# domkirke/acids_transforms

Hardware: AMD Instinct MI355X
Metric: spectrogram frames/sec (fwd+invert), n_fft=1024 hop=256 (higher is better)
Workload: dtype f32; 1 GPU; configs[1]: batch=1024 clips/GPU x 4 s mono 44.1 kHz, STFT fwd + Magnitude(mel=128, log1p, unipolar) [one fused kernel] + ISTFT invert, fp32; n_fft=1024, hop=256, frames_per_clip=690, clips_per_gpu=1024

## Files before the change

acids_transforms_amd/csrc/capi.hip:

```cpp
#include <hip/hip_runtime.h>
#include <math.h>
#include <stdint.h>
#include <vector>

#include "../../include/acids_hip.h"
#include "autograd.h"
#include "band_bank.h"
#include "fft512.h"
#include "stft_launch.h"

#include <atomic>
#include "variants.h"
namespace at_hip {
constexpr int kMaxDevices = 16;
static float2* g_twiddles[kMaxDevices] = {nullptr};
static float2* g_side[kMaxDevices] = {nullptr};

static bool device_tables(const float2*& tw, const float2*& side) {
  int dev = 0;
  if (hipGetDevice(&dev) != hipSuccess || dev < 0 || dev >= kMaxDevices || !g_twiddles[dev]) return false;
  tw = g_twiddles[dev];
  side = g_side[dev];
  return true;
}

static bool is_pow2(int n) { return n > 0 && (n & (n - 1)) == 0; }
static bool fft_size_ok(int n) { return n >= 2 && n <= 16384 && (!(n & 1) || n < 8192); }
static bool fft_mixed(int n) { return !is_pow2(n) || n < 8; }

__global__ void envelope_table_kernel(const float* w, int n_fft, int hop, int R, float* env) {
  int i = blockIdx.x * blockDim.x + threadIdx.x;
  if (i >= (1 << R) * hop) return;
  int mask = i / hop, r = i - mask * hop;
  float s = 0.f;
  for (int q = 0; q < R; ++q)
    if (mask & (1 << q)) {
      int o = hop * (R - 1 - q) + r;
      if (o < n_fft) s += w[o] * w[o];
    }
  env[i] = s;
}
static std::atomic<int> g_variants[kVarCount];
int variant(int which) { return g_variants[which].load(std::memory_order_relaxed); }
}

using namespace at_hip;

extern "C" {

int at_abi_version(void) { return 4; }

int at_set_variant(int which, int value) {
  if (which < 0 || which >= kVarCount || value < 0 || value > (which >= kVarFirstPlan ? 65535 : 4)) return AT_EINVAL;
  g_variants[which].store(value, std::memory_order_relaxed);
  return AT_OK;
}

int at_get_variant(int which) {
  if (which < 0 || which >= kVarCount) return AT_EINVAL;
  return g_variants[which].load(std::memory_order_relaxed);
}

const char* at_error_string(int code) {
  switch (code) {
    case AT_OK: return "ok";
    case AT_EINVAL: return "invalid argument";
    case AT_EUNSUPPORTED: return "unsupported configuration";
    case AT_ENOTINIT: return "at_init() not called for this device";
    case AT_EWORKSPACE: return "workspace too small";
    case AT_ELAUNCH: return "HIP launch/runtime error";
    default: return "unknown error";
  }
}

int at_init(int device) {
  if (device < 0 || device >= kMaxDevices) return AT_EINVAL;
  if (g_twiddles[device]) return AT_OK;
  int prev = 0;
  if (hipGetDevice(&prev) != hipSuccess) return AT_ELAUNCH;
  if (hipSetDevice(device) != hipSuccess) return AT_ELAUNCH;
  std::vector<float2> tab(kTwiddleCount);
  const double two_pi = 6.283185307179586476925286766559;
  for (int k = 1; k < 8; ++k)
    for (int l = 0; l < 64; ++l) {
      double a1 = -two_pi * (double)(l * k) / 512.0;
      tab[(k - 1) * 64 + l] = make_float2((float)cos(a1), (float)sin(a1));
      double a2 = -two_pi * (double)((l & 7) * k) / 64.0;
      tab[(7 + k - 1) * 64 + l] = make_float2((float)cos(a2), (float)sin(a2));
    }
  for (int m = 0; m < 8; ++m)
    for (int l = 0; l < 64; ++l) {
      double a = -two_pi * (double)(l + 64 * m) / 1024.0;
      tab[(14 + m) * 64 + l] = make_float2((float)cos(a), (float)sin(a));
    }
  float2* d = nullptr;
  int rc = AT_OK;
  if (hipMalloc((void**)&d, sizeof(float2) * (kTwiddleCount + kTileCtrSlots)) != hipSuccess) rc = AT_ELAUNCH;
  if (rc == AT_OK && hipMemcpy(d, tab.data(), sizeof(float2) * kTwiddleCount, hipMemcpyHostToDevice) != hipSuccess)
    rc = AT_ELAUNCH;
  if (rc == AT_OK && hipMemset(d + kTwiddleCount, 0, sizeof(float2) * kTileCtrSlots) != hipSuccess) rc = AT_ELAUNCH;
  float2* d2 = nullptr;
  if (rc == AT_OK) {
    std::vector<float2> t2(kSideTableCount);
    auto fill = [&](int at, int count, int r, double n) {
      for (int k = 0; k < count; ++k) {
        const double a = -two_pi * (double)(r * k) / n;
        t2[at + k] = make_float2((float)cos(a), (float)sin(a));
      }
    };
    fill(kSideW2048, 1024, 1, 2048.0);
    fill(kSideW512, 256, 1, 512.0);
    for (int r = 1; r < 4; ++r) fill(kSide256 + (r - 1) * 128, 128, r, 512.0);
    for (int r = 1; r < 8; ++r) fill(kSide128 + (r - 1) * 64, 64, r, 512.0);
    fill(kSide4096, 2048, 1, 4096.0);
    for (int r = 1; r < 4; ++r) fill(kSide4096Radix + (r - 1) * 512, 512, r, 2048.0);
    if (hipMalloc((void**)&d2, sizeof(float2) * t2.size()) != hipSuccess) rc = AT_ELAUNCH;
    if (rc == AT_OK && hipMemcpy(d2, t2.data(), sizeof(float2) * t2.size(), hipMemcpyHostToDevice) != hipSuccess)
      rc = AT_ELAUNCH;
  }
  if (rc == AT_OK) {
    g_side[device] = d2;
    g_twiddles[device] = d;
  }
  (void)hipSetDevice(prev);
  return rc;
}

int at_stft_forward(const float* x, int64_t B, int64_t L, int64_t clip_stride, int64_t T, int n_fft, int hop,
                    int center, const float* window, float* out_complex, float* phase, void* stream) {
  if (B < 0 || T < 0 || L < 0 || hop <= 0 || n_fft <= 0) return AT_EINVAL;
  if (B * T == 0) return AT_OK;
  if (!x || !window || !out_complex) return AT_EINVAL;
  if (!fft_size_ok(n_fft)) return AT_EUNSUPPORTED;
  if (center && L <= n_fft / 2) return AT_EINVAL;
  hipStream_t s = (hipStream_t)stream;
  const uintptr_t walign = (uintptr_t)window;
  const float2 *tw = nullptr, *side = nullptr;
  if (n_fft == 1024 && (walign & 7) == 0) {
    if (!device_tables(tw, side)) return AT_ENOTINIT;
    if ((hop == 256 || hop == 128 || hop == 512) && center && (clip_stride & 1) == 0)
      return launch_stft1024_h256_fwd(x, B, L, clip_stride, T, window, tw, (float2*)out_complex, phase, nullptr,
                                      nullptr, nullptr, nullptr, 0.f, 0, 0, 0, s, nullptr, hop);
    return launch_stft1024_fwd(x, B, L, clip_stride, T, hop, center, window, tw, (float2*)out_complex, phase, s);
  }
  if (n_fft == 2048 && (walign & 15) == 0) {
    if (!device_tables(tw, side)) return AT_ENOTINIT;
    return launch_stft2048_fwd(x, B, L, clip_stride, T, hop, center, window, tw, side + kSideW2048, (float2*)out_complex,
                               phase, s);
  }
  if (n_fft == 4096 && (walign & 15) == 0) {
    if (!device_tables(tw, side)) return AT_ENOTINIT;
    return launch_stft4096_fwd(x, B, L, clip_stride, T, hop, center, window, tw, side + kSide4096, (float2*)out_complex,
                               phase, s);
  }
  if ((n_fft == 256 || n_fft == 128) && (walign & 7) == 0) {
    if (!device_tables(tw, side)) return AT_ENOTINIT;
    return launch_stft_small_fwd(n_fft, x, B, L, clip_stride, T, hop, center, window, tw,
                                 side + (n_fft == 256 ? kSide256 : kSide128), (float2*)out_complex, phase, s);
  }
  if (n_fft == 512 && (walign & 7) == 0) {
    if (!device_tables(tw, side)) return AT_ENOTINIT;
    return launch_stft512_fwd(x, B, L, clip_stride, T, hop, center, window, tw, side + kSideW512, (float2*)out_complex,
                              phase, s);
  }
  if (fft_mixed(n_fft))
    return launch_rfft_mixed(x, B, L, clip_stride, T, n_fft, hop, center, window, (float2*)out_complex, phase, s);
  return launch_rfft_generic(x, B, L, clip_stride, T, n_fft, hop, center, window, (float2*)out_complex, phase, s);
}

int at_stft_mel_forward(const float* x, int64_t B, int64_t L, int64_t clip_stride, int64_t T, int n_fft, int hop,
                        const float* window, const int32_t* lane_filter, const int32_t* lane_start,
                        const float* band_weights, int n_filters, int n_passes, const int32_t* pass_len_host,
                        int contrast, int power2, const float* offset, const float* scale, float eps,
                        float* out_complex_or_null, float* phase_or_null, float* feat, int feat_channel_major,
                        void* stream) {
  if (B < 0 || T < 0 || L < 0) return AT_EINVAL;
// ... 403 lines not shown
```

acids_transforms_amd/csrc/fft512.h:

```cpp
#pragma once
#include <hip/hip_runtime.h>
#include <stdint.h>

#include "fastmath.h"

namespace at_hip {

#ifndef AT_WAVE_PRIORITY
#define AT_WAVE_PRIORITY 1
#endif
template <int LEVEL>
__device__ __forceinline__ void wave_priority() {
#if AT_WAVE_PRIORITY
  __builtin_amdgcn_s_setprio(LEVEL);
#endif
}

constexpr int kFftLdsFloat2PerWave = 568;

constexpr int kTwiddleCount = 22 * 64;
constexpr int kTileCtrSlots = 4096;

__device__ __forceinline__ float2 cadd(float2 a, float2 b) { return make_float2(a.x + b.x, a.y + b.y); }

typedef float v2f __attribute__((ext_vector_type(2)));

__device__ __forceinline__ v2f to_v(float2 a) { return (v2f){a.x, a.y}; }
__device__ __forceinline__ float2 to_f2(v2f a) { return make_float2(a.x, a.y); }

__device__ __forceinline__ v2f add_mi(v2f a, v2f b) {
  v2f r;
  asm("v_pk_add_f32 %0, %1, %2 op_sel:[0,1] op_sel_hi:[1,0] neg_hi:[0,1]" : "=v"(r) : "v"(a), "v"(b));
  return r;
}
__device__ __forceinline__ v2f add_pi(v2f a, v2f b) {
  v2f r;
  asm("v_pk_add_f32 %0, %1, %2 op_sel:[0,1] op_sel_hi:[1,0] neg_lo:[0,1]" : "=v"(r) : "v"(a), "v"(b));
  return r;
}
__device__ __forceinline__ v2f fma_mi(v2f a, v2f b, v2f rr) {
  v2f r;
  asm("v_pk_fma_f32 %0, %1, %2, %3 op_sel:[1,0,0] op_sel_hi:[0,1,1] neg_hi:[1,0,0]" : "=v"(r) : "v"(b), "s"(rr), "v"(a));
  return r;
}
__device__ __forceinline__ v2f fma_pi(v2f a, v2f b, v2f rr) {
  v2f r;
  asm("v_pk_fma_f32 %0, %1, %2, %3 op_sel:[1,0,0] op_sel_hi:[0,1,1] neg_lo:[1,0,0]" : "=v"(r) : "v"(b), "s"(rr), "v"(a));
  return r;
}
template <bool INV> __device__ __forceinline__ v2f rot_add(v2f a, v2f b) { return INV ? add_pi(a, b) : add_mi(a, b); }
template <bool INV> __device__ __forceinline__ v2f rot_sub(v2f a, v2f b) { return INV ? add_mi(a, b) : add_pi(a, b); }
template <bool INV> __device__ __forceinline__ v2f rot_fma(v2f a, v2f b, v2f rr) { return INV ? fma_pi(a, b, rr) : fma_mi(a, b, rr); }
template <bool INV> __device__ __forceinline__ v2f rot_fms(v2f a, v2f b, v2f rr) { return INV ? fma_mi(a, b, rr) : fma_pi(a, b, rr); }

__device__ __forceinline__ v2f cmul_v(v2f a, v2f w) {
  const v2f t = a.yy * w.yx;
  v2f r;
  asm("v_pk_fma_f32 %0, %1, %2, %3 op_sel_hi:[0,1,1] neg_lo:[0,0,1]" : "=v"(r) : "v"(a), "v"(w), "v"(t));
  return r;
}
__device__ __forceinline__ v2f cmul_conj_v(v2f a, v2f w) {
  const v2f t = a.yy * w.yx;
  v2f r;
  asm("v_pk_fma_f32 %0, %1, %2, %3 op_sel_hi:[0,1,1] neg_hi:[0,1,0]" : "=v"(r) : "v"(a), "v"(w), "v"(t));
  return r;
}
template <bool INV> __device__ __forceinline__ v2f twiddle(v2f a, v2f w) { return INV ? cmul_conj_v(a, w) : cmul_v(a, w); }
__device__ __forceinline__ v2f add_conj(v2f a, v2f b) {
  v2f r;
  asm("v_pk_add_f32 %0, %1, %2 neg_hi:[0,1]" : "=v"(r) : "v"(a), "v"(b));
  return r;
}
__device__ __forceinline__ v2f sub_conj(v2f a, v2f b) {
  v2f r;
  asm("v_pk_add_f32 %0, %1, %2 neg_lo:[0,1]" : "=v"(r) : "v"(a), "v"(b));
  return r;
}
__device__ __forceinline__ v2f scale_add_mi(v2f a, v2f hh, v2f b) {
  v2f r;
  asm("v_pk_fma_f32 %0, %1, %2, %3 op_sel:[0,0,1] op_sel_hi:[1,1,0] neg_hi:[0,0,1]" : "=v"(r) : "v"(a), "s"(hh), "v"(b));
  return r;
}

template <bool INV>
__device__ __forceinline__ void radix8(v2f (&v)[8]) {
  const v2f rr = {0.70710678118654752440f, 0.70710678118654752440f};
  const v2f a0 = v[0] + v[4], a4 = v[0] - v[4];
  const v2f a1 = v[1] + v[5], d1 = v[1] - v[5];
  const v2f a2 = v[2] + v[6], d2 = v[2] - v[6];
  const v2f a3 = v[3] + v[7], d3 = v[3] - v[7];
  const v2f s5 = rot_add<INV>(d1, d1);
  const v2f s7 = rot_sub<INV>(d3, d3);
  const v2f b0 = a0 + a2, b2 = a0 - a2;
  const v2f b1 = a1 + a3, d13 = a1 - a3;
  const v2f b4 = rot_add<INV>(a4, d2), b6 = rot_sub<INV>(a4, d2);
  const v2f u5 = s5 - s7, u7 = s5 + s7;
  v[0] = b0 + b1;
  v[4] = b0 - b1;
  v[2] = rot_add<INV>(b2, d13);
  v[6] = rot_sub<INV>(b2, d13);
  v[1] = __builtin_elementwise_fma(u5, rr, b4);
  v[5] = __builtin_elementwise_fma(-u5, rr, b4);
  v[3] = rot_fma<INV>(b6, u7, rr);
  v[7] = rot_fms<INV>(b6, u7, rr);
}

#ifndef AT_LDS_NOMERGE
#define AT_LDS_NOMERGE 1
#endif
template <typename T>
__device__ __forceinline__ T lds_read_single(const T* p) {
#if AT_LDS_NOMERGE
  typedef const volatile __attribute__((address_space(3))) T* lds_ptr;
  return *(lds_ptr)(p);
#else
  return *p;
#endif
}

__device__ __forceinline__ void wave_lds_sync() {
  __builtin_amdgcn_fence(__ATOMIC_RELEASE, "wavefront");
  __builtin_amdgcn_wave_barrier();
  __builtin_amdgcn_fence(__ATOMIC_ACQUIRE, "wavefront");
}

struct Twiddles {
  v2f t1[7];
  v2f t2[7];
  v2f tr[8];
  __device__ __forceinline__ v2f get1(int k) const { return t1[k]; }
  __device__ __forceinline__ v2f get2(int k) const { return t2[k]; }
  __device__ __forceinline__ v2f getr(int m) const { return tr[m]; }
};

template <bool INV>
struct LdsTwiddles {
  const float2* tab;
  int lane;
  __device__ __forceinline__ v2f get1(int k) const { return lds_read_single(reinterpret_cast<const v2f*>(tab) + k * 64 + lane); }
  __device__ __forceinline__ v2f get2(int k) const { return lds_read_single(reinterpret_cast<const v2f*>(tab) + (7 + k) * 64 + lane); }
  __device__ __forceinline__ v2f getr(int m) const { return lds_read_single(reinterpret_cast<const v2f*>(tab) + (14 + m) * 64 + lane); }
};
struct HybridTwiddles {
  v2f t1[7];
  v2f t2[7];
  const float2* tab;
  int col;
  __device__ __forceinline__ v2f get1(int k) const { return t1[k]; }
  __device__ __forceinline__ v2f get2(int k) const { return t2[k]; }
  __device__ __forceinline__ v2f getr(int m) const { return lds_read_single(reinterpret_cast<const v2f*>(tab) + (14 + m) * 64 + col); }
};

template <bool INV>
__device__ __forceinline__ float2 twiddle_for_lds(const float2* __restrict__ tab, int i) {
  const float2 a = tab[i];
  return (!INV && i >= 14 * 64) ? make_float2(0.5f * a.x, 0.5f * a.y) : a;
}

template <bool INV>
__device__ __forceinline__ void load_twiddles(Twiddles& tw, const float2* __restrict__ tab, int lane) {
#pragma unroll
  for (int k = 0; k < 7; ++k) {
    tw.t1[k] = to_v(tab[k * 64 + lane]);
    tw.t2[k] = to_v(tab[(7 + k) * 64 + lane]);
  }
#pragma unroll
  for (int m = 0; m < 8; ++m) tw.tr[m] = to_v(twiddle_for_lds<INV>(tab, (14 + m) * 64 + lane));
}

#ifndef AT_XCHG1_SWAP
#define AT_XCHG1_SWAP 1
#endif
__device__ __forceinline__ void xchg1_registers(v2f (&v)[8]) {
#pragma unroll
  for (int k = 0; k < 4; ++k)
#pragma unroll
    for (int c = 0; c < 2; ++c) {
      const auto sw = __builtin_amdgcn_permlane32_swap(__float_as_uint(v[k][c]), __float_as_uint(v[k + 4][c]), false, false);
      v[k][c] = __uint_as_float(sw[0]);
      v[k + 4][c] = __uint_as_float(sw[1]);
    }
#pragma unroll
  for (int g = 0; g < 8; g += 4)
#pragma unroll
    for (int k = g; k < g + 2; ++k)
#pragma unroll
      for (int c = 0; c < 2; ++c) {
        const auto sw = __builtin_amdgcn_permlane16_swap(__float_as_uint(v[k][c]), __float_as_uint(v[k + 2][c]), false, false);
        v[k][c] = __uint_as_float(sw[0]);
        v[k + 2][c] = __uint_as_float(sw[1]);
      }
#pragma unroll
  for (int k = 0; k < 8; k += 2)
#pragma unroll
    for (int c = 0; c < 2; ++c) {
      const int a = __float_as_int(v[k][c]), b = __float_as_int(v[k + 1][c]);
      const int a2 = __builtin_amdgcn_update_dpp(a, b, 0x128, 0xf, 0xc, false);
      const int b2 = __builtin_amdgcn_update_dpp(b, a, 0x128, 0xf, 0x3, false);
      v[k][c] = __int_as_float(a2);
      v[k + 1][c] = __int_as_float(b2);
    }
}

template <bool INV, typename TW>
__device__ __forceinline__ void fft512(v2f (&v)[8], const TW& tw, float2* lds_f2, int lane, int out_lane = -1) {
  if (out_lane < 0) out_lane = lane;
  v2f* lds = reinterpret_cast<v2f*>(lds_f2);
  const int lo = lane & 7, hi = lane >> 3;
  radix8<INV>(v);
#pragma unroll
  for (int k = 1; k < 8; ++k) v[k] = twiddle<INV>(v[k], tw.get1(k - 1));
  if constexpr (AT_XCHG1_SWAP == 2 || (AT_XCHG1_SWAP == 1 && !INV)) {
    xchg1_registers(v);
  } else {
#pragma unroll
    for (int k = 0; k < 8; ++k) lds[hi * 72 + lo + 8 * k] = v[k];
    wave_lds_sync();
#pragma unroll
    for (int k = 0; k < 8; ++k) v[k] = lds_read_single(lds + k * 72 + lane);
    wave_lds_sync();
  }
  radix8<INV>(v);
#pragma unroll
  for (int k = 1; k < 8; ++k) v[k] = twiddle<INV>(v[k], tw.get2(k - 1));
#pragma unroll
  for (int k = 0; k < 8; ++k) lds[lo * 66 + hi + 8 * k] = v[k];
  wave_lds_sync();
#pragma unroll
  for (int k = 0; k < 8; ++k) v[k] = lds_read_single(lds + k * 66 + out_lane);
  wave_lds_sync();
  radix8<INV>(v);
}
constexpr bool fft512_exchanges_cover(int lo_slot, int hi_slot) {
  for (int s = lo_slot; s <= hi_slot; ++s) {
    bool hit = false;
    for (int a = 0; a < 8 && !hit; ++a) {
      if (s >= a * 72 && s < a * 72 + 64) hit = true;
      if (s >= a * 66 && s < a * 66 + 64) hit = true;
    }
    if (!hit) return false;
  }
  return true;
}
static_assert(AT_XCHG1_SWAP || (fft512_exchanges_cover(256, 319) && 320 <= kFftLdsFloat2PerWave),
              "the fixed-length mel epilogue reads absrow[513..639] uncleared: both exchanges must rewrite float2 slots 256..319");

template <bool INV, typename TW>
__device__ __forceinline__ void fft512(float2 (&f)[8], const TW& tw, float2* lds, int lane) {
  v2f v[8];
#pragma unroll
  for (int m = 0; m < 8; ++m) v[m] = to_v(f[m]);
  fft512<INV>(v, tw, lds, lane);
#pragma unroll
  for (int m = 0; m < 8; ++m) f[m] = to_f2(v[m]);
}

template <int Q>
__device__ __forceinline__ void mirror_regs_rot(const v2f (&v)[Q], v2f (&p)[Q], int lane, int rot, int col) {
  const int src = (2 * rot - lane) & 63;
  v2f q[Q];
#pragma unroll
  for (int m = 0; m < Q; ++m) {
    q[m].x = __shfl(v[m].x, src, 64);
    q[m].y = __shfl(v[m].y, src, 64);
  }
#pragma unroll
  for (int m = 0; m < Q; ++m) {
    const v2f a = q[Q - 1 - m];
    const v2f b = q[(Q - m) % Q];
    p[m] = (col == 0) ? b : a;
  }
}
template <int Q>
__device__ __forceinline__ void mirror_regs(const v2f (&v)[Q], v2f (&p)[Q], int lane) {
  mirror_regs_rot<Q>(v, p, lane, 0, lane);
}

template <typename TW>
__device__ __forceinline__ void rfft_merge(v2f (&v)[8], const TW& tw, int lane, float2& nyq) {
  const v2f hh = {0.5f, 0.5f};
  v2f p[8];
  mirror_regs<8>(v, p, lane);
  nyq = make_float2(v[0].x - v[0].y, 0.0f);
#pragma unroll
  for (int m = 0; m < 8; ++m) {
    const v2f e = add_conj(v[m], p[m]);
    const v2f d = sub_conj(v[m], p[m]);
    const v2f wd = cmul_v(d, tw.getr(m));
    v[m] = scale_add_mi(e, hh, wd);
  }
}
template <typename TW>
__device__ __forceinline__ void rfft_merge_rot(v2f (&v)[8], const TW& tw, int lane, int rot, int col, float2& nyq) {
  const v2f hh = {0.5f, 0.5f};
  v2f p[8];
  mirror_regs_rot<8>(v, p, lane, rot, col);
  nyq = make_float2(v[0].x - v[0].y, 0.0f);
#pragma unroll
  for (int m = 0; m < 8; ++m) {
    const v2f e = add_conj(v[m], p[m]);
    const v2f d = sub_conj(v[m], p[m]);
    const v2f wd = cmul_v(d, tw.getr(m));
    v[m] = scale_add_mi(e, hh, wd);
  }
}
template <typename TW>
__device__ __forceinline__ void rfft_merge(float2 (&f)[8], const TW& tw, int lane, float2& nyq) {
  v2f v[8];
#pragma unroll
  for (int m = 0; m < 8; ++m) v[m] = to_v(f[m]);
  rfft_merge(v, tw, lane, nyq);
#pragma unroll
  for (int m = 0; m < 8; ++m) f[m] = to_f2(v[m]);
}

template <typename TW>
__device__ __forceinline__ void irfft_split(v2f (&v)[8], const TW& tw, int lane, float xnyq_re) {
  if (lane == 0) v[0].y = 0.0f;
  v2f p[8];
  mirror_regs<8>(v, p, lane);
  if (lane == 0) p[0] = (v2f){xnyq_re, 0.0f};
#pragma unroll
  for (int m = 0; m < 8; ++m) {
    const v2f e = add_conj(v[m], p[m]);
    const v2f d = cmul_conj_v(sub_conj(v[m], p[m]), tw.getr(m));
    v[m] = add_pi(e, d);
  }
}
template <typename TW>
__device__ __forceinline__ void irfft_split(float2 (&f)[8], const TW& tw, int lane, float xnyq_re) {
  v2f v[8];
#pragma unroll
  for (int m = 0; m < 8; ++m) v[m] = to_v(f[m]);
  irfft_split(v, tw, lane, xnyq_re);
#pragma unroll
  for (int m = 0; m < 8; ++m) f[m] = to_f2(v[m]);
}

template <int K, typename P>
__device__ __forceinline__ void load_shared_frame(const P& p, long long b, long long t, int lane, float2 (&q)[8]) {
  constexpr int N = 1024 / K, PER = 64 / K;
  if (t >= p.T) {
#pragma unroll
    for (int j = 0; j < 8; ++j) q[j] = make_float2(0.f, 0.f);
    return;
  }
  const float* clip = p.x + b * p.clip_stride;
  const long long start = t * (long long)p.hop - (p.center ? N / 2 : 0);
  const bool interior = (start >= 0) && (start + N <= p.L);
  const int u = lane / K;
  if (interior && ((((uintptr_t)(clip + start)) & 7) == 0)) {
    const float2* src = reinterpret_cast<const float2*>(clip + start);
#pragma unroll
    for (int j = 0; j < 8; ++j) q[j] = src[u + PER * j];
  } else {
#pragma unroll
    for (int j = 0; j < 8; ++j) {
      const long long i0 = start + 2 * (u + PER * j);
      float v[2];
#pragma unroll
      for (int c = 0; c < 2; ++c) {
        const long long i = i0 + c;
        if (interior) v[c] = clip[i];
        else if (p.center) v[c] = clip[reflect_index(i, p.L)];
        else v[c] = (i >= 0 && i < p.L) ? clip[i] : 0.0f;
      }
      q[j] = make_float2(v[0], v[1]);
    }
  }
}

}
```

acids_transforms_amd/csrc/stft1024.hip:

```cpp
#include <hip/hip_runtime.h>
#include "fastmath.h"
#include <type_traits>
#include <stdint.h>
#include <stdlib.h>
#include <stdio.h>
#include <string.h>
#include <atomic>

#include "band_bank.h"
#include "fft512.h"
#include "fwd1024_forms.h"
#include "run_plan.h"
#include "stft_launch.h"
#include "variants.h"

#ifndef AT_ISTFT_NT
#define AT_ISTFT_NT 1
#endif
#ifndef AT_ISTFT_NTLOAD
#define AT_ISTFT_NTLOAD 1
#endif

namespace at_hip {

// ... 582 lines not shown
      float2 fresh[HS];
#pragma unroll
      for (int k = 0; k < HS; ++k) fresh[k] = nsrc[64 * k];
      nsrc += H / 2;
      frame_body(fresh);
    }
  }
  for (; t < t1; ++t) {
    flush_nyquist();
    float2 fresh[HS];
#pragma unroll
    for (int k = 0; k < HS; ++k) fresh[k] = make_float2(0.f, 0.f);
    if (t + 1 < t1) {
#pragma unroll
      for (int k = 0; k < HS; ++k) {
        const long long i0 = t * H + 512 + 128 * k;
        fresh[k] = load_pair(clip, L, i0, i0 >= 0 && i0 + 128 <= L, clip_aligned, lane2);
      }
    }
    frame_body(fresh);
  }
  flush_nyquist();
  if constexpr (AL) {
    if (lane < rot) put(sp, carry);
  }
  if constexpr (FQP != 0) {
    wave_lds_sync();
    const float* fbuf = reinterpret_cast<const float*>(lds) - 2 * kFeatCarry;
    const float4 v = reinterpret_cast<const float4*>(fbuf)[lane];
    const float vv[4] = {v.x, v.y, v.z, v.w};
#pragma unroll
    for (int c = 0; c < 4; ++c)
      if (4 * lane + c < fc && 4 * lane + c >= fhead) fdst[4 * lane + c] = vv[c];
    wave_lds_sync();
  }
  };

  if constexpr (!PW) {
    do_run((long long)blockIdx.x * FWD_WAVES + wave, true);
  } else {
    for (int it = 0;; ++it) {
      const unsigned tile = __builtin_amdgcn_readfirstlane(s_tile[it & 1]);
      if (tile >= p.n_tiles) break;
      unsigned nxt = 0;
      if (threadIdx.x == 0) nxt = atomicAdd(p.tile_ctr, 1u);
      do_run((long long)tile * FWD_WAVES + wave, false);
      if (threadIdx.x == 0) s_tile[(it + 1) & 1] = nxt;
      __syncthreads();
    }
    if (threadIdx.x == 0) {
      if (atomicAdd(p.tile_ctr + 1, 1u) == gridDim.x - 1) {
        atomicExch(p.tile_ctr, 0u);
        atomicExch(p.tile_ctr + 1, 0u);
      }
    }
  }
}

enum { IN_COMPLEX = 0, IN_POLAR = 1, IN_GL = 2 };
enum { OUT_OLA = 0, OUT_FRAMES = 1 };

struct InvParams {
  const float2* X;
  const float* mag;
  const float* phase;
  const float2* tprev;
  float gl_mom;
  const float* window;
  const float* env;
  const float2* tw;
  float* y;
  long long B, T;
  long long runs_per_clip;
  long long slots_per_run;
  long long total_frames, frames_per_block;
};

typedef float f32x2 __attribute__((ext_vector_type(2)));
template <int IN_MODE>
struct RawFrame;
template <>
struct RawFrame<IN_COMPLEX> {
  f32x2 d[8];
  float ny0;
};
template <>
struct RawFrame<IN_POLAR> {
  float a[8], ph[8];
  float ny0, ny1;
};
template <>
struct RawFrame<IN_GL> {
  f32x2 r[8], t[8];
  float a[8];
  f32x2 rny, tny;
  float any;
};

__device__ __forceinline__ void load_raw(const InvParams& p, long long f, int lane, RawFrame<IN_COMPLEX>& q) {
  const f32x2* row = reinterpret_cast<const f32x2*>(p.X + f * F);
#pragma unroll
  for (int m = 0; m < 8; ++m) {
#if AT_ISTFT_NTLOAD
    q.d[m] = __builtin_nontemporal_load(row + lane + 64 * m);
#else
    q.d[m] = row[lane + 64 * m];
#endif
  }
  q.ny0 = reinterpret_cast<const float*>(row + 512)[0];
}
__device__ __forceinline__ void load_raw(const InvParams& p, long long f, int lane, RawFrame<IN_POLAR>& q) {
  const float* mrow = p.mag + f * F;
  const float* prow = p.phase + f * F;
#pragma unroll
  for (int m = 0; m < 8; ++m) {
    q.a[m] = mrow[lane + 64 * m];
    q.ph[m] = prow[lane + 64 * m];
  }
  q.ny0 = mrow[512];
  q.ny1 = prow[512];
}

__device__ __forceinline__ void load_raw(const InvParams& p, long long f, int lane, RawFrame<IN_GL>& q) {
  const f32x2* rrow = reinterpret_cast<const f32x2*>(p.X + f * F);
  const f32x2* trow = reinterpret_cast<const f32x2*>(p.tprev + f * F);
  const float* mrow = p.mag + f * F;
#pragma unroll
  for (int m = 0; m < 8; ++m) {
    q.r[m] = rrow[lane + 64 * m];
    q.t[m] = trow[lane + 64 * m];
    q.a[m] = mrow[lane + 64 * m];
  }
  q.rny = rrow[512];
  q.tny = trow[512];
  q.any = mrow[512];
}

__device__ __forceinline__ float2 gl_update(f32x2 r, f32x2 t, float mag, float mom) {
  float ax = r.x, ay = r.y;
  ax -= mom * t.x;
  ay -= mom * t.y;
  const float d = __builtin_amdgcn_sqrtf(fmaf(ax, ax, ay * ay)) + 1e-16f;
  const float s = mag * __builtin_amdgcn_rcpf(d);
  return make_float2(s * ax, s * ay);
}

__device__ __forceinline__ void raw_to_spectrum(const RawFrame<IN_COMPLEX>& q, float2 (&v)[8], float& nyq_re) {
#pragma unroll
  for (int m = 0; m < 8; ++m) v[m] = make_float2(q.d[m].x, q.d[m].y);
  nyq_re = q.ny0;
}
__device__ __forceinline__ void raw_to_spectrum(const RawFrame<IN_POLAR>& q, float2 (&v)[8], float& nyq_re) {
#pragma unroll
  for (int m = 0; m < 8; ++m) {
    float sn, cs;
    fast_sincosf(q.ph[m], sn, cs);
    v[m] = make_float2(q.a[m] * cs, q.a[m] * sn);
  }
  float sn, cs;
  fast_sincosf(q.ny1, sn, cs);
  nyq_re = q.ny0 * cs;
}

__device__ __forceinline__ void raw_to_spectrum(const RawFrame<IN_GL>& q, float2 (&v)[8], float& nyq_re, float mom) {
#pragma unroll
  for (int m = 0; m < 8; ++m) v[m] = gl_update(q.r[m], q.t[m], q.a[m], mom);
  nyq_re = gl_update(q.rny, q.tny, q.any, mom).x;
}

template <int IN_MODE>
__device__ __forceinline__ void load_spectrum(const InvParams& p, long long f, int lane, float2 (&v)[8], float& nyq_re) {
  RawFrame<IN_MODE> q;
  load_raw(p, f, lane, q);
  raw_to_spectrum(q, v, nyq_re);
}

__device__ __forceinline__ float2 scaled_window(const float* window, int i) {
  const float2 w = reinterpret_cast<const float2*>(window)[i];
  return make_float2(w.x * (1.0f / 1024.0f), w.y * (1.0f / 1024.0f));
}

template <typename TW>
__device__ __forceinline__ void synth_frame_nowin(const float2 (&v)[8], float nyq_re, const TW& tw, float2* lds, int lane,
                                                  v2f (&z)[8]) {
#pragma unroll
  for (int m = 0; m < 8; ++m) z[m] = to_v(v[m]);
  irfft_split(z, tw, lane, nyq_re);
  fft512<true>(z, tw, lds, lane);
}
__device__ __forceinline__ v2f ola_window(const float2* win, int lane, int m) {
  return lds_read_single(reinterpret_cast<const v2f*>(win) + lane + 64 * m);
}

template <typename TW>
__device__ __forceinline__ void synth_frame(float2 (&v)[8], float nyq_re, const TW& tw, const float2* win,
                                            float2* lds, int lane) {
  v2f z[8];
#pragma unroll
  for (int m = 0; m < 8; ++m) z[m] = to_v(v[m]);
  irfft_split(z, tw, lane, nyq_re);
  fft512<true>(z, tw, lds, lane);
#pragma unroll
  for (int m = 0; m < 8; ++m) {
    const v2f w = lds_read_single(reinterpret_cast<const v2f*>(win) + lane + 64 * m);
    v[m] = to_f2(z[m] * w);
  }
}

template <int IN_MODE, int DEPTH, bool TWLDS, int HS = 2>
__global__ __launch_bounds__(64 * WAVES_PER_BLOCK, IN_MODE == IN_GL ? 2 : (TWLDS ? 5 : 4) - DEPTH) void istft1024_ola_kernel(InvParams p) {
  constexpr int R = 8 / HS;
  constexpr int C = 4 / HS;
  constexpr int H = 128 * HS;
  constexpr int kFull = (1 << R) - 1;
  __shared__ float2 lds_all[WAVES_PER_BLOCK * kFftLdsFloat2PerWave + 512 + (TWLDS ? kTwiddleCount : 0)];
  const int lane = threadIdx.x & 63;
  const int wave = __builtin_amdgcn_readfirstlane(threadIdx.x >> 6);
  float2* lds = lds_all + wave * kFftLdsFloat2PerWave;
  float2* win = lds_all + WAVES_PER_BLOCK * kFftLdsFloat2PerWave;
  float2* twtab = win + 512;
  for (int i = threadIdx.x; i < 512; i += 64 * WAVES_PER_BLOCK) win[i] = scaled_window(p.window, i);
  if (TWLDS)
    for (int i = threadIdx.x; i < kTwiddleCount; i += 64 * WAVES_PER_BLOCK) twtab[i] = p.tw[i];
  __syncthreads();

  const long long run = (long long)blockIdx.x * WAVES_PER_BLOCK + wave;
  const long long b = run / p.runs_per_clip;
  if (b >= p.B) return;
  const long long r = run - b * p.runs_per_clip;
  const long long nslots = p.T - 1;
  const long long j0 = r * p.slots_per_run;
  long long j1 = j0 + p.slots_per_run;
  if (j1 > nslots) j1 = nslots;
  if (j0 >= j1) return;

  Twiddles tw_regs;
  if (!TWLDS) load_twiddles<true>(tw_regs, p.tw, lane);
  const LdsTwiddles<true> tw_lds = {twtab, lane};
  auto synth = [&](const float2 (&v)[8], float nyq, v2f (&z)[8]) {
    if (TWLDS) synth_frame_nowin(v, nyq, tw_lds, lds, lane, z);
    else synth_frame_nowin(v, nyq, tw_regs, lds, lane, z);
  };

  v2f acc[8];
#pragma unroll
  for (int m = 0; m < 8; ++m) acc[m] = (v2f){0.f, 0.f};

  const long long fbase = b * p.T;
  float* yclip = p.y + b * (H * nslots);
  long long t = (j0 + C - (R - 1) > 0) ? j0 + C - (R - 1) : 0;
  const long long t_last = j1 - 1 + C;
  const long long t_have = (t_last < p.T - 1) ? t_last : p.T - 1;

  RawFrame<IN_MODE> q0 = {}, q1 = {};
  if (t <= t_have) load_raw(p, fbase + t, lane, q0);
  if (t + 1 <= t_have) load_raw(p, fbase + t + 1, lane, q1);

  auto consume = [&](const RawFrame<IN_MODE>& q) {
    float2 v[8];
    float nyq;
    if constexpr (IN_MODE == IN_GL) raw_to_spectrum(q, v, nyq, p.gl_mom);
    else raw_to_spectrum(q, v, nyq);
    v2f z[8];
    synth(v, nyq, z);
#pragma unroll
    for (int m = 0; m < 8; ++m) acc[m] = __builtin_elementwise_fma(z[m], ola_window(win, lane, m), acc[m]);
  };
  auto put_y = [&](float2* dst, float2 val) {
#if AT_ISTFT_NT
    __builtin_nontemporal_store((v2f){val.x, val.y}, reinterpret_cast<v2f*>(dst));
#else
    *dst = val;
#endif
  };
  static_assert(sizeof(v2f) == sizeof(float2), "");
  auto emit = [&](long long j, const float2* env) {
    float2* dst = reinterpret_cast<float2*>(yclip + j * H);
#pragma unroll
    for (int k = 0; k < HS; ++k) {
      const float2 e = env[lane + 64 * k];
      put_y(dst + lane + 64 * k, make_float2(acc[k].x / e.x, acc[k].y / e.y));
    }
  };
  float2 rcp[HS];
  auto emit_fast = [&](long long j) {
    float2* dst = reinterpret_cast<float2*>(yclip + j * H);
#pragma unroll
    for (int k = 0; k < HS; ++k) put_y(dst + lane + 64 * k, make_float2(acc[k].x * rcp[k].x, acc[k].y * rcp[k].y));
  };
  auto advance = [&]() {
#pragma unroll
    for (int m = 0; m < 8 - HS; ++m) acc[m] = acc[m + HS];
#pragma unroll
    for (int m = 8 - HS; m < 8; ++m) acc[m] = (v2f){0.f, 0.f};
  };
  {
    const float2* env_full = reinterpret_cast<const float2*>(p.env + kFull * H);
#pragma unroll
    for (int k = 0; k < HS; ++k) {
      const float2 e = env_full[lane + 64 * k];
      rcp[k] = make_float2(1.0f / e.x, 1.0f / e.y);
    }
  }
  auto generic_step = [&]() {
    if (t <= t_have) {
      const RawFrame<IN_MODE> cur = q0;
      q0 = q1;
      if (t + 2 <= t_have) load_raw(p, fbase + t + 2, lane, q1);
      consume(cur);
    }
    const long long j = t - C;
    if (j >= j0 && j < j1) {
      int mask = 0;
#pragma unroll
      for (int q = 0; q < R; ++q) {
        const long long tt = t - (R - 1) + q;
        if (tt >= 0 && tt < p.T) mask |= 1 << q;
      }
      if (mask == kFull) emit_fast(j);
      else emit(j, reinterpret_cast<const float2*>(p.env + mask * H));
    }
    advance();
    ++t;
  };

  long long fast_begin = j0 + C > R - 1 ? j0 + C : R - 1;
  long long fast_end = (j1 - 1 + C < t_have - 2) ? j1 - 1 + C : t_have - 2;
  while (t < fast_begin && t <= t_last) generic_step();
  if (t <= fast_end) {
    if (DEPTH == 2) {
      auto fast_step = [&](RawFrame<IN_MODE>& q) {
        const RawFrame<IN_MODE> cur = q;
        load_raw(p, fbase + t + 2, lane, q);
        consume(cur);
        emit_fast(t - C);
        advance();
        ++t;
      };
      while (t + 1 <= fast_end) {
        fast_step(q0);
        fast_step(q1);
      }
    } else {
      q1 = {};
      for (; t <= fast_end; ++t) {
        const RawFrame<IN_MODE> cur = q0;
        load_raw(p, fbase + t + 1, lane, q0);
        consume(cur);
        emit_fast(t - C);
        advance();
      }
      q1 = {};
      if (t + 1 <= t_have) load_raw(p, fbase + t + 1, lane, q1);
    }
  }
  while (t <= t_last) generic_step();
}

template <int IN_MODE, int NW, int OCC>
__global__ __launch_bounds__(64 * NW, OCC) void istft1024_tile_kernel(InvParams p) {
  constexpr int HS = 2, R = 4, H = 256;
  constexpr int kFull = (1 << R) - 1;
  static_assert(IN_MODE != IN_GL, "the Griffin-Lim form keeps the long-run kernel");
  __shared__ float2 lds_all[NW * kFftLdsFloat2PerWave + 512];
  __shared__ float4 park_all[NW * 6 * 64];
  const int lane = threadIdx.x & 63;
  const int wave = __builtin_amdgcn_readfirstlane(threadIdx.x >> 6);
  float2* lds = lds_all + wave * kFftLdsFloat2PerWave;
  float2* win = lds_all + NW * kFftLdsFloat2PerWave;

  const long long tile = blockIdx.x;
  const long long b = tile / p.runs_per_clip;
  const long long k = tile - b * p.runs_per_clip;
  const long long n = p.slots_per_run;
  const long long T = p.T;
  const long long tile0 = k * p.frames_per_block;
  long long tile1 = tile0 + p.frames_per_block;
  if (tile1 > T) tile1 = T;
  auto share = [&](int w, long long& a, long long& e) {
    a = tile0 + w * n;
    if (a > tile1) a = tile1;
    e = (w == NW - 1) ? tile1 : a + n;
    if (e > tile1) e = tile1;
  };
  long long ta, tb;
  share(wave, ta, tb);
  bool self_cool = true;
  if (wave < NW - 1) {
    long long a2, e2;
    share(wave + 1, a2, e2);
    self_cool = e2 - a2 < 3;
  }
  long long t_stop = (self_cool && tb > ta) ? tb + 3 : tb;
  if (t_stop > T) t_stop = T;
  const bool parks = wave > 0 && ta > 0;
  const long long pe0 = ta == 0 ? 2 : ta + 3;
  const long long pe1 = tb + 3;

  const long long fbase = b * T;
  float* yclip = p.y + b * (H * (T - 1));
  long long t = ta;
  RawFrame<IN_MODE> q0 = {}, q1 = {};
  if (t < t_stop) load_raw(p, fbase + t, lane, q0);
  if (t + 1 < t_stop) load_raw(p, fbase + t + 1, lane, q1);

  for (int i = threadIdx.x; i < 512; i += 64 * NW) win[i] = scaled_window(p.window, i);
  Twiddles tw;
  load_twiddles<true>(tw, p.tw, lane);
  __syncthreads();

  v2f acc[8];
#pragma unroll
  for (int m = 0; m < 8; ++m) acc[m] = (v2f){0.f, 0.f};
  auto consume = [&](const RawFrame<IN_MODE>& q, v2f (&z)[8]) {
    float2 v[8];
    float nyq;
    raw_to_spectrum(q, v, nyq);
    synth_frame_nowin(v, nyq, tw, lds, lane, z);
#pragma unroll
    for (int m = 0; m < 8; ++m) acc[m] = __builtin_elementwise_fma(z[m], ola_window(win, lane, m), acc[m]);
  };
  auto put_y = [&](float2* dst, float2 val) {
    __builtin_nontemporal_store((v2f){val.x, val.y}, reinterpret_cast<v2f*>(dst));
  };
  float2 rcp[HS];
  {
    const float2* env_full = reinterpret_cast<const float2*>(p.env + kFull * H);
#pragma unroll
    for (int kk = 0; kk < HS; ++kk) {
      const float2 e = env_full[lane + 64 * kk];
      rcp[kk] = make_float2(1.0f / e.x, 1.0f / e.y);
    }
  }
  auto emit_regs = [&](long long hp, v2f a0, v2f a1) {
    float2* dst = reinterpret_cast<float2*>(yclip + (hp - 2) * H);
    if (hp >= 3 && hp < T) {
      put_y(dst + lane, make_float2(a0.x * rcp[0].x, a0.y * rcp[0].y));
      put_y(dst + lane + 64, make_float2(a1.x * rcp[1].x, a1.y * rcp[1].y));
    } else {
      int mask = 0;
#pragma unroll
      for (int q = 0; q < R; ++q) {
        const long long tt = hp - (R - 1) + q;
        if (tt >= 0 && tt < T) mask |= 1 << q;
      }
      const float2* env = reinterpret_cast<const float2*>(p.env + mask * H);
      const float2 e0 = env[lane], e1 = env[lane + 64];
      put_y(dst + lane, make_float2(a0.x / e0.x, a0.y / e0.y));
      put_y(dst + lane + 64, make_float2(a1.x / e1.x, a1.y / e1.y));
    }
  };
  auto advance = [&]() {
#pragma unroll
    for (int m = 0; m < 8 - HS; ++m) acc[m] = acc[m + HS];
#pragma unroll
    for (int m = 8 - HS; m < 8; ++m) acc[m] = (v2f){0.f, 0.f};
  };
  float4* park = park_all + wave * 6 * 64 + lane;
  auto generic_step = [&]() {
    const RawFrame<IN_MODE> cur = q0;
    q0 = q1;
    if (t + 2 < t_stop) load_raw(p, fbase + t + 2, lane, q1);
    v2f v[8];
    consume(cur, v);
    const long long i = t - ta;
    if (parks && i < 3 && t < tb) {
      const int base = i == 0 ? 0 : (i == 1 ? 3 : 5);
#pragma unroll
      for (int s = 0; s < 3; ++s)
        if (s < 3 - i) park[(base + s) * 64] = make_float4(v[2 * s].x, v[2 * s].y, v[2 * s + 1].x, v[2 * s + 1].y);
    }
    if (t >= pe0 && t < pe1) emit_regs(t, acc[0], acc[1]);
    advance();
    ++t;
  };

  long long fast_begin = ta + 3 > pe0 ? ta + 3 : pe0;
  if (fast_begin < 3) fast_begin = 3;
  long long fast_end = tb - 1;
  if (fast_end > t_stop - 3) fast_end = t_stop - 3;
  while (t < fast_begin && t < tb) generic_step();
  if (t <= fast_end) {
    auto fast_step = [&](RawFrame<IN_MODE>& q) {
      const RawFrame<IN_MODE> cur = q;
      load_raw(p, fbase + t + 2, lane, q);
      v2f v[8];
      consume(cur, v);
      float2* dst = reinterpret_cast<float2*>(yclip + (t - 2) * H);
      put_y(dst + lane, make_float2(acc[0].x * rcp[0].x, acc[0].y * rcp[0].y));
      put_y(dst + lane + 64, make_float2(acc[1].x * rcp[1].x, acc[1].y * rcp[1].y));
      advance();
      ++t;
    };
    while (t + 1 <= fast_end) {
      fast_step(q0);
      fast_step(q1);
    }
  }
  while (t < tb) generic_step();
  __syncthreads();
  if (self_cool) {
    while (t < t_stop) generic_step();
    if (t_stop == T && T >= pe0 && T < pe1 && t == T) emit_regs(T, acc[0], acc[1]);
  } else if (tb > ta) {
    const float4* nx = park_all + (wave + 1) * 6 * 64 + lane;
    auto add4 = [&](int hop, int s, const float4 pc) {
      acc[2 * hop] = __builtin_elementwise_fma((v2f){pc.x, pc.y}, ola_window(win, lane, 2 * s), acc[2 * hop]);
      acc[2 * hop + 1] = __builtin_elementwise_fma((v2f){pc.z, pc.w}, ola_window(win, lane, 2 * s + 1), acc[2 * hop + 1]);
    };
    add4(0, 0, nx[0 * 64]);
    add4(1, 1, nx[1 * 64]);
    add4(1, 0, nx[3 * 64]);
    add4(2, 2, nx[2 * 64]);
    add4(2, 1, nx[4 * 64]);
    add4(2, 0, nx[5 * 64]);
#pragma unroll
    for (int s = 0; s < 3; ++s)
      if (tb + s >= pe0) emit_regs(tb + s, acc[2 * s], acc[2 * s + 1]);
  }
}

template <int IN_MODE>
__global__ __launch_bounds__(64 * WAVES_PER_BLOCK) void irfft1024_frames_kernel(InvParams p) {
  __shared__ float2 lds_all[WAVES_PER_BLOCK * kFftLdsFloat2PerWave + 512];
  const int lane = threadIdx.x & 63;
  const int wave = threadIdx.x >> 6;
  float2* lds = lds_all + wave * kFftLdsFloat2PerWave;
  float2* win = lds_all + WAVES_PER_BLOCK * kFftLdsFloat2PerWave;
  for (int i = threadIdx.x; i < 512; i += 64 * WAVES_PER_BLOCK) win[i] = scaled_window(p.window, i);
  __syncthreads();
  Twiddles tw;
  load_twiddles<true>(tw, p.tw, lane);
  const long long f_begin = (long long)blockIdx.x * p.frames_per_block;
  long long f_end = f_begin + p.frames_per_block;
  if (f_end > p.total_frames) f_end = p.total_frames;
  for (long long f = f_begin + wave; f < f_end; f += WAVES_PER_BLOCK) {
    float2 v[8];
    float nyq;
    load_spectrum<IN_MODE>(p, f, lane, v, nyq);
    synth_frame(v, nyq, tw, win, lds, lane);
    float2* dst = reinterpret_cast<float2*>(p.y + f * N);
#pragma unroll
    for (int m = 0; m < 8; ++m) dst[lane + 64 * m] = v[m];
  }
}

}

namespace at_hip {

struct FwdFormEntry {
  void (*kernel)(FwdRunParams);
  const char* name;
  int waves;
  int packed_lds_bytes;
  bool persistent;
};
template <class Form> constexpr FwdFormEntry fwd_form_entry(const char* name) {
  return {stft1024_h256_fwd_kernel<Form>, name, Form::waves, fwd1024::packed_lds_bytes<Form>(), Form::persistent};
}
static const FwdFormEntry kFwdForms[] = {
#define X(F) fwd_form_entry<fwd1024::F>(#F),
    AT_FWD1024_FORMS(X)
#ifdef AT_DEV_SWITCHES
    AT_FWD1024_DEV_FORMS(X)
#endif
#undef X
};
#ifdef AT_DEV_SWITCHES
static_assert(sizeof(kFwdForms) / sizeof(kFwdForms[0]) == kFwd1024Forms, "one entry per form");
#else
static_assert(sizeof(kFwdForms) / sizeof(kFwdForms[0]) == kFwd1024ProductForms, "one entry per product form; no switch picks a dev form here");
#endif

unsigned* tile_counter_slot(const float2* tw) {
  static std::atomic<unsigned> cursor{0};
  const unsigned slot = cursor.fetch_add(1, std::memory_order_relaxed) % kTileCtrSlots;
  return reinterpret_cast<unsigned*>(const_cast<float2*>(tw) + kTwiddleCount) + 2 * slot;
}

int launch_stft1024_fwd(const float* x, long long B, long long L, long long clip_stride, long long T, int hop,
                        int center, const float* window, const float2* tw, float2* out, float* phase,
                        hipStream_t stream) {
  FwdParams p;
  p.x = x; p.window = window; p.tw = tw; p.out = out; p.phase = phase;
  p.B = B; p.L = L; p.clip_stride = clip_stride; p.T = T; p.hop = hop; p.center = center;
  p.total_frames = B * T;
  if (p.total_frames == 0) return 0;
  long long max_blocks = (long long)num_cus() * 4;
  long long fpb = (p.total_frames + max_blocks - 1) / max_blocks;
  fpb = ((fpb + WAVES_PER_BLOCK - 1) / WAVES_PER_BLOCK) * WAVES_PER_BLOCK;
  if (fpb < 2 * WAVES_PER_BLOCK) fpb = 2 * WAVES_PER_BLOCK;
  p.frames_per_block = fpb;
  long long blocks = (p.total_frames + fpb - 1) / fpb;
  if (phase)
    hipLaunchKernelGGL(stft1024_fwd_kernel<true>, dim3((unsigned)blocks), dim3(64 * WAVES_PER_BLOCK), 0, stream, p);
  else
    hipLaunchKernelGGL(stft1024_fwd_kernel<false>, dim3((unsigned)blocks), dim3(64 * WAVES_PER_BLOCK), 0, stream, p);
  return hipGetLastError() == hipSuccess ? 0 : -5;
}

int launch_stft1024_h256_fwd(const float* x, long long B, long long L, long long clip_stride, long long T,
                             const float* window, const float2* tw, float2* out, float* phase, const BandBank* bank,
                             float* feat, const float* offset, const float* scale, float eps, int contrast, int power2,
                             int feat_channel_major, hipStream_t stream, const PolarOut* polar, int hop) {
  Fwd1024Call call = {};
  call.hop = hop;
  call.spectrum = out; call.phase = phase; call.polar = polar; call.channel_major = feat_channel_major;
  call.bank = bank;
  if (bank) { call.n_passes = bank->n_passes; call.n_filters = bank->n_filters; call.pass_len = bank->pass_len; }
  call.contrast = contrast; call.power2 = power2;
  call.out_aligned_512 = (((uintptr_t)out) & 511) == 0; call.feat_aligned_16 = (((uintptr_t)feat) & 15) == 0;
  call.epilogue = variant(kVarEpilogue);
  static const int store_mode = [] {
    const char* e = dev_env("ACIDS_FWD_STORES");
    return !e ? 2 : !strcmp(e, "rows") ? 0 : !strcmp(e, "aligned") ? 1 : 2;
  }();
  static const bool pw_mode = [] { const char* e = dev_env("ACIDS_FWD_PW"); return e && e[0] == '1'; }();
  call.dev_stores = store_mode; call.dev_persistent = pw_mode;
  if (const char* e = dev_env("ACIDS_FWD_HYB")) call.dev_register_tables = atoi(e);
  call.dev_no_register_tables = dev_env("ACIDS_FWD_NOHYB");
  const int form_id = pick_fwd1024(call);
  if (form_id < 0 || form_id >= (int)(sizeof(kFwdForms) / sizeof(kFwdForms[0]))) return -1;
// ... 146 lines not shown
```

Before: 473.0 million frames/s.

## Load inverse spectrum in mirror-paired order to pair bins within each lane

The inverse real-FFT split step now loads bins so that registers m and 7-m in a lane hold mirror partners (k and 512-k). Both outputs of each pair are computed locally, which replaces the full cross-lane mirror exchange with four shuffled registers per frame plus special handling of bin 256 on lane 0. The Nyquist-only scalar becomes the self-paired middle bin. This trades fewer cross-lane exchange operations for reversed, less coalesced loads on half the registers and some extra lane-0 register shuffling.

After: 485.4 million frames/s (median of 6 runs). +2.6%, better.

```diff
diff --git a/acids_transforms_amd/csrc/capi.hip b/acids_transforms_amd/csrc/capi.hip
--- a/acids_transforms_amd/csrc/capi.hip
+++ b/acids_transforms_amd/csrc/capi.hip
@@ -90,8 +90,8 @@
     }
   for (int m = 0; m < 8; ++m)
     for (int l = 0; l < 64; ++l) {
-      double a = -two_pi * (double)(l + 64 * m) / 1024.0;
-      tab[(14 + m) * 64 + l] = make_float2((float)cos(a), (float)sin(a));
+      float2& w = tab[(14 + m) * 64 + l];
+      inv1024::w1024(l + 64 * m, w.x, w.y);
     }
   float2* d = nullptr;
   int rc = AT_OK;
diff --git a/acids_transforms_amd/csrc/fft512.h b/acids_transforms_amd/csrc/fft512.h
--- a/acids_transforms_amd/csrc/fft512.h
+++ b/acids_transforms_amd/csrc/fft512.h
@@ -3,6 +3,7 @@
 #include <stdint.h>
 
 #include "fastmath.h"
+#include "inv1024_pairs.h"
 
 namespace at_hip {
 
@@ -74,6 +75,11 @@
 __device__ __forceinline__ v2f sub_conj(v2f a, v2f b) {
   v2f r;
   asm("v_pk_add_f32 %0, %1, %2 neg_lo:[0,1]" : "=v"(r) : "v"(a), "v"(b));
+  return r;
+}
+__device__ __forceinline__ v2f conj_add_mi(v2f a, v2f b) {
+  v2f r;
+  asm("v_pk_add_f32 %0, %1, %2 op_sel:[0,1] op_sel_hi:[1,0] neg_hi:[1,0]" : "=v"(r) : "v"(a), "v"(b));
   return r;
 }
 __device__ __forceinline__ v2f scale_add_mi(v2f a, v2f hh, v2f b) {
@@ -128,9 +134,11 @@
   v2f t1[7];
   v2f t2[7];
   v2f tr[8];
+  v2f tr_self;
   __device__ __forceinline__ v2f get1(int k) const { return t1[k]; }
   __device__ __forceinline__ v2f get2(int k) const { return t2[k]; }
   __device__ __forceinline__ v2f getr(int m) const { return tr[m]; }
+  __device__ __forceinline__ v2f getr_self() const { return tr_self; }
 };
 
 template <bool INV>
@@ -140,6 +148,7 @@
   __device__ __forceinline__ v2f get1(int k) const { return lds_read_single(reinterpret_cast<const v2f*>(tab) + k * 64 + lane); }
   __device__ __forceinline__ v2f get2(int k) const { return lds_read_single(reinterpret_cast<const v2f*>(tab) + (7 + k) * 64 + lane); }
   __device__ __forceinline__ v2f getr(int m) const { return lds_read_single(reinterpret_cast<const v2f*>(tab) + (14 + m) * 64 + lane); }
+  __device__ __forceinline__ v2f getr_self() const { return lds_read_single(reinterpret_cast<const v2f*>(tab) + (14 + inv1024::kSelfPairedRow) * 64); }
 };
 struct HybridTwiddles {
   v2f t1[7];
@@ -166,6 +175,11 @@
   }
 #pragma unroll
   for (int m = 0; m < 8; ++m) tw.tr[m] = to_v(twiddle_for_lds<INV>(tab, (14 + m) * 64 + lane));
+  if (INV) {
+    const float2 w = tab[(14 + inv1024::kSelfPairedRow) * 64];
+    tw.tr_self = (v2f){__int_as_float(__builtin_amdgcn_readfirstlane(__float_as_int(w.x))),
+                       __int_as_float(__builtin_amdgcn_readfirstlane(__float_as_int(w.y)))};
+  }
 }
 
 #ifndef AT_XCHG1_SWAP
@@ -315,24 +329,40 @@
 }
 
 template <typename TW>
-__device__ __forceinline__ void irfft_split(v2f (&v)[8], const TW& tw, int lane, float xnyq_re) {
-  if (lane == 0) v[0].y = 0.0f;
-  v2f p[8];
-  mirror_regs<8>(v, p, lane);
-  if (lane == 0) p[0] = (v2f){xnyq_re, 0.0f};
-#pragma unroll
-  for (int m = 0; m < 8; ++m) {
-    const v2f e = add_conj(v[m], p[m]);
-    const v2f d = cmul_conj_v(sub_conj(v[m], p[m]), tw.getr(m));
+__device__ __forceinline__ void irfft_split(v2f (&v)[8], const TW& tw, int lane, v2f x256) {
+  if (lane == 0) {
+    v[0].y = 0.0f;
+    v[7].y = 0.0f;
+  }
+#pragma unroll
+  for (int m = 0; m < inv1024::kPairs; ++m) {
+    const int n = inv1024::partner_reg(m);
+    const v2f e = add_conj(v[m], v[n]);
+    const v2f d = cmul_conj_v(sub_conj(v[m], v[n]), tw.getr(m));
     v[m] = add_pi(e, d);
+    v[n] = conj_add_mi(e, d);
+  }
+  if (lane == 0) {
+    const v2f e = add_conj(x256, x256);
+    const v2f d = cmul_conj_v(sub_conj(x256, x256), tw.getr_self());
+    v[7] = v[6];
+    v[6] = v[5];
+    v[5] = v[4];
+    v[4] = add_pi(e, d);
+  }
+  const int src = inv1024::exchange_lane(lane);
+#pragma unroll
+  for (int m = inv1024::kPairs; m < 8; ++m) {
+    v[m].x = __shfl(v[m].x, src, 64);
+    v[m].y = __shfl(v[m].y, src, 64);
   }
 }
 template <typename TW>
-__device__ __forceinline__ void irfft_split(float2 (&f)[8], const TW& tw, int lane, float xnyq_re) {
+__device__ __forceinline__ void irfft_split(float2 (&f)[8], const TW& tw, int lane, float2 x256) {
   v2f v[8];
 #pragma unroll
   for (int m = 0; m < 8; ++m) v[m] = to_v(f[m]);
-  irfft_split(v, tw, lane, xnyq_re);
+  irfft_split(v, tw, lane, to_v(x256));
 #pragma unroll
   for (int m = 0; m < 8; ++m) f[m] = to_f2(v[m]);
 }
diff --git a/acids_transforms_amd/csrc/inv1024_pairs.h b/acids_transforms_amd/csrc/inv1024_pairs.h
--- /dev/null
+++ b/acids_transforms_amd/csrc/inv1024_pairs.h
@@ -0,0 +1,40 @@
+#pragma once
+#include <math.h>
+
+namespace at_hip {
+namespace inv1024 {
+
+inline void w1024(int k, float& re, float& im) {
+  const double a = -6.283185307179586476925286766559 * (double)k / 1024.0;
+  re = (float)cos(a);
+  im = (float)sin(a);
+}
+
+constexpr int kLanes = 64, kRegs = 8, kPairs = 4;
+constexpr int kSelfPairedBin = 256;
+constexpr int kSelfPairedRow = 4;
+
+constexpr int load_start(int lane, int m) { return m < kPairs ? lane : 64 - lane; }
+constexpr int load_step(int m) { return 64 * m; }
+constexpr int load_bin(int lane, int m) { return load_start(lane, m) + load_step(m); }
+constexpr int partner_reg(int m) { return kRegs - 1 - m; }
+constexpr int exchange_lane(int lane) { return (64 - lane) & 63; }
+constexpr int twiddle_bin(int lane, int m) { return lane + 64 * m; }
+
+constexpr int rotated_bin(int lane, int m) {
+  return (lane == 0 && m >= kPairs) ? (m == kPairs ? kSelfPairedBin : load_bin(0, m - 1)) : load_bin(lane, m);
+}
+constexpr int final_bin(int lane, int m) { return m < kPairs ? rotated_bin(lane, m) : rotated_bin(exchange_lane(lane), m); }
+
+constexpr bool pairs_and_order_hold() {
+  for (int lane = 0; lane < kLanes; ++lane)
+    for (int m = 0; m < kRegs; ++m) {
+      if (load_bin(lane, m) + load_bin(lane, partner_reg(m)) != 512) return false;
+      if (final_bin(lane, m) != lane + 64 * m) return false;
+    }
+  return true;
+}
+static_assert(pairs_and_order_hold(), "registers m and 7 - m are mirror partners; fft512<true> gets Z[lane + 64 m]");
+
+}
+}
diff --git a/acids_transforms_amd/csrc/stft1024.hip b/acids_transforms_amd/csrc/stft1024.hip
--- a/acids_transforms_amd/csrc/stft1024.hip
+++ b/acids_transforms_amd/csrc/stft1024.hip
@@ -688,19 +688,19 @@
 template <>
 struct RawFrame<IN_COMPLEX> {
   f32x2 d[8];
-  float ny0;
+  f32x2 mid;
 };
 template <>
 struct RawFrame<IN_POLAR> {
   float a[8], ph[8];
-  float ny0, ny1;
+  float mid0, mid1;
 };
 template <>
 struct RawFrame<IN_GL> {
   f32x2 r[8], t[8];
   float a[8];
-  f32x2 rny, tny;
-  float any;
+  f32x2 rmid, tmid;
+  float amid;
 };
 
 __device__ __forceinline__ void load_raw(const InvParams& p, long long f, int lane, RawFrame<IN_COMPLEX>& q) {
@@ -708,23 +708,23 @@
 #pragma unroll
   for (int m = 0; m < 8; ++m) {
 #if AT_ISTFT_NTLOAD
-    q.d[m] = __builtin_nontemporal_load(row + lane + 64 * m);
+    q.d[m] = __builtin_nontemporal_load(row + inv1024::load_start(lane, m) + inv1024::load_step(m));
 #else
-    q.d[m] = row[lane + 64 * m];
+    q.d[m] = (row + inv1024::load_start(lane, m))[inv1024::load_step(m)];
 #endif
   }
-  q.ny0 = reinterpret_cast<const float*>(row + 512)[0];
+  q.mid = row[inv1024::kSelfPairedBin];
 }
 __device__ __forceinline__ void load_raw(const InvParams& p, long long f, int lane, RawFrame<IN_POLAR>& q) {
   const float* mrow = p.mag + f * F;
   const float* prow = p.phase + f * F;
 #pragma unroll
   for (int m = 0; m < 8; ++m) {
-    q.a[m] = mrow[lane + 64 * m];
-    q.ph[m] = prow[lane + 64 * m];
-  }
-  q.ny0 = mrow[512];
-  q.ny1 = prow[512];
+    q.a[m] = (mrow + inv1024::load_start(lane, m))[inv1024::load_step(m)];
+    q.ph[m] = (prow + inv1024::load_start(lane, m))[inv1024::load_step(m)];
+  }
+  q.mid0 = mrow[inv1024::kSelfPairedBin];
+  q.mid1 = prow[inv1024::kSelfPairedBin];
 }
 
 __device__ __forceinline__ void load_raw(const InvParams& p, long long f, int lane, RawFrame<IN_GL>& q) {
@@ -733,13 +733,13 @@
   const float* mrow = p.mag + f * F;
 #pragma unroll
   for (int m = 0; m < 8; ++m) {
-    q.r[m] = rrow[lane + 64 * m];
-    q.t[m] = trow[lane + 64 * m];
-    q.a[m] = mrow[lane + 64 * m];
-  }
-  q.rny = rrow[512];
-  q.tny = trow[512];
-  q.any = mrow[512];
+    q.r[m] = (rrow + inv1024::load_start(lane, m))[inv1024::load_step(m)];
+    q.t[m] = (trow + inv1024::load_start(lane, m))[inv1024::load_step(m)];
+    q.a[m] = (mrow + inv1024::load_start(lane, m))[inv1024::load_step(m)];
+  }
+  q.rmid = rrow[inv1024::kSelfPairedBin];
+  q.tmid = trow[inv1024::kSelfPairedBin];
+  q.amid = mrow[inv1024::kSelfPairedBin];
 }
 
 __device__ __forceinline__ float2 gl_update(f32x2 r, f32x2 t, float mag, float mom) {
@@ -751,12 +751,12 @@
   return make_float2(s * ax, s * ay);
 }
 
-__device__ __forceinline__ void raw_to_spectrum(const RawFrame<IN_COMPLEX>& q, float2 (&v)[8], float& nyq_re) {
+__device__ __forceinline__ void raw_to_spectrum(const RawFrame<IN_COMPLEX>& q, float2 (&v)[8], float2& x256) {
 #pragma unroll
   for (int m = 0; m < 8; ++m) v[m] = make_float2(q.d[m].x, q.d[m].y);
-  nyq_re = q.ny0;
-}
-__device__ __forceinline__ void raw_to_spectrum(const RawFrame<IN_POLAR>& q, float2 (&v)[8], float& nyq_re) {
+  x256 = make_float2(q.mid.x, q.mid.y);
+}
+__device__ __forceinline__ void raw_to_spectrum(const RawFrame<IN_POLAR>& q, float2 (&v)[8], float2& x256) {
 #pragma unroll
   for (int m = 0; m < 8; ++m) {
     float sn, cs;
@@ -764,21 +764,21 @@
     v[m] = make_float2(q.a[m] * cs, q.a[m] * sn);
   }
   float sn, cs;
-  fast_sincosf(q.ny1, sn, cs);
-  nyq_re = q.ny0 * cs;
-}
-
-__device__ __forceinline__ void raw_to_spectrum(const RawFrame<IN_GL>& q, float2 (&v)[8], float& nyq_re, float mom) {
+  fast_sincosf(q.mid1, sn, cs);
+  x256 = make_float2(q.mid0 * cs, q.mid0 * sn);
+}
+
+__device__ __forceinline__ void raw_to_spectrum(const RawFrame<IN_GL>& q, float2 (&v)[8], float2& x256, float mom) {
 #pragma unroll
   for (int m = 0; m < 8; ++m) v[m] = gl_update(q.r[m], q.t[m], q.a[m], mom);
-  nyq_re = gl_update(q.rny, q.tny, q.any, mom).x;
+  x256 = gl_update(q.rmid, q.tmid, q.amid, mom);
 }
 
 template <int IN_MODE>
-__device__ __forceinline__ void load_spectrum(const InvParams& p, long long f, int lane, float2 (&v)[8], float& nyq_re) {
+__device__ __forceinline__ void load_spectrum(const InvParams& p, long long f, int lane, float2 (&v)[8], float2& x256) {
   RawFrame<IN_MODE> q;
   load_raw(p, f, lane, q);
-  raw_to_spectrum(q, v, nyq_re);
+  raw_to_spectrum(q, v, x256);
 }
 
 __device__ __forceinline__ float2 scaled_window(const float* window, int i) {
@@ -787,11 +787,11 @@
 }
 
 template <typename TW>
-__device__ __forceinline__ void synth_frame_nowin(const float2 (&v)[8], float nyq_re, const TW& tw, float2* lds, int lane,
+__device__ __forceinline__ void synth_frame_nowin(const float2 (&v)[8], float2 x256, const TW& tw, float2* lds, int lane,
                                                   v2f (&z)[8]) {
 #pragma unroll
   for (int m = 0; m < 8; ++m) z[m] = to_v(v[m]);
-  irfft_split(z, tw, lane, nyq_re);
+  irfft_split(z, tw, lane, to_v(x256));
   fft512<true>(z, tw, lds, lane);
 }
 __device__ __forceinline__ v2f ola_window(const float2* win, int lane, int m) {
@@ -799,12 +799,12 @@
 }
 
 template <typename TW>
-__device__ __forceinline__ void synth_frame(float2 (&v)[8], float nyq_re, const TW& tw, const float2* win,
+__device__ __forceinline__ void synth_frame(float2 (&v)[8], float2 x256, const TW& tw, const float2* win,
                                             float2* lds, int lane) {
   v2f z[8];
 #pragma unroll
   for (int m = 0; m < 8; ++m) z[m] = to_v(v[m]);
-  irfft_split(z, tw, lane, nyq_re);
+  irfft_split(z, tw, lane, to_v(x256));
   fft512<true>(z, tw, lds, lane);
 #pragma unroll
   for (int m = 0; m < 8; ++m) {
@@ -843,9 +843,9 @@
   Twiddles tw_regs;
   if (!TWLDS) load_twiddles<true>(tw_regs, p.tw, lane);
   const LdsTwiddles<true> tw_lds = {twtab, lane};
-  auto synth = [&](const float2 (&v)[8], float nyq, v2f (&z)[8]) {
-    if (TWLDS) synth_frame_nowin(v, nyq, tw_lds, lds, lane, z);
-    else synth_frame_nowin(v, nyq, tw_regs, lds, lane, z);
+  auto synth = [&](const float2 (&v)[8], float2 x256, v2f (&z)[8]) {
+    if (TWLDS) synth_frame_nowin(v, x256, tw_lds, lds, lane, z);
+    else synth_frame_nowin(v, x256, tw_regs, lds, lane, z);
   };
 
   v2f acc[8];
@@ -864,11 +864,11 @@
 
   auto consume = [&](const RawFrame<IN_MODE>& q) {
     float2 v[8];
-    float nyq;
-    if constexpr (IN_MODE == IN_GL) raw_to_spectrum(q, v, nyq, p.gl_mom);
-    else raw_to_spectrum(q, v, nyq);
+    float2 x256;
+    if constexpr (IN_MODE == IN_GL) raw_to_spectrum(q, v, x256, p.gl_mom);
+    else raw_to_spectrum(q, v, x256);
     v2f z[8];
-    synth(v, nyq, z);
+    synth(v, x256, z);
 #pragma unroll
     for (int m = 0; m < 8; ++m) acc[m] = __builtin_elementwise_fma(z[m], ola_window(win, lane, m), acc[m]);
   };
@@ -1020,9 +1020,9 @@
   for (int m = 0; m < 8; ++m) acc[m] = (v2f){0.f, 0.f};
   auto consume = [&](const RawFrame<IN_MODE>& q, v2f (&z)[8]) {
     float2 v[8];
-    float nyq;
-    raw_to_spectrum(q, v, nyq);
-    synth_frame_nowin(v, nyq, tw, lds, lane, z);
+    float2 x256;
+    raw_to_spectrum(q, v, x256);
+    synth_frame_nowin(v, x256, tw, lds, lane, z);
 #pragma unroll
     for (int m = 0; m < 8; ++m) acc[m] = __builtin_elementwise_fma(z[m], ola_window(win, lane, m), acc[m]);
   };
@@ -1142,9 +1142,9 @@
   if (f_end > p.total_frames) f_end = p.total_frames;
   for (long long f = f_begin + wave; f < f_end; f += WAVES_PER_BLOCK) {
     float2 v[8];
-    float nyq;
-    load_spectrum<IN_MODE>(p, f, lane, v, nyq);
-    synth_frame(v, nyq, tw, win, lds, lane);
+    float2 x256;
+    load_spectrum<IN_MODE>(p, f, lane, v, x256);
+    synth_frame(v, x256, tw, win, lds, lane);
     float2* dst = reinterpret_cast<float2*>(p.y + f * N);
 #pragma unroll
     for (int m = 0; m < 8; ++m) dst[lane + 64 * m] = v[m];
```
